# d3sm0/gym_pomdp

Hardware: AMD Instinct MI355X
Metric: env steps/sec (whole node), RockSample(7,8) batch=2^20, 1/2/4/8 MI355X (higher is better)
Workload: dtype int32

## Files before the change

### gym_pomdp_amd/csrc/envs/rock.hip.h

```cpp
#pragma once
#include "../envs_common.hip.h"

namespace pomdp {

template <int W, bool STOCH = false>
struct RockEnv {
    using Params = pomdp_rock_params;
    using Reward = int32_t;
    using S = typename std::conditional<W == 1, uint32_t, uint64_t>::type;
    static constexpr int WORDS = W;
    static constexpr const char *NAME = STOCH ? (W == 1 ? "StochasticRockEnv<1>" : "StochasticRockEnv<2>") : (W == 1 ? "RockEnv<1>" : "RockEnv<2>");
    static constexpr bool POOLED_LPT2 = !STOCH;
    static constexpr bool QUAD_STEP = true;
    static constexpr bool HAS_ROCKS = true;
    static constexpr bool POOLED_ANY_LPT = !STOCH;
    static constexpr bool STOCHASTIC = STOCH;
    static constexpr bool QUAD_TAB = true;
    struct Shared {
        uint2 thr[32];
        int8_t grid[256];
        uint8_t rxy[16];
        uint16_t rpos[16];
        uint32_t dir_y[16];
        uint32_t dir_x[16];
// ... 324 lines not shown
        const int penalty = STOCH ? 0 : -100;
        const int id = sh.grid[x * 16 + y];
        const int sh_ = 8 + 2 * (id & 15);
        const uint32_t code = (uint32_t)(s >> sh_) & 3u;
        const bool sample_ok = ((uint32_t)id < K) & (code != 1u);
        const uint32_t a2 = (uint32_t)a << 1;
        const uint32_t nx = x + (uint32_t)__builtin_amdgcn_sbfe(0xC4, a2, 2u), ny = y + (uint32_t)__builtin_amdgcn_sbfe(0x31, a2, 2u);
        const bool inside = max(nx, ny) < size;
        const bool is_move = a < 4, is_sample = a == 4, east = a == 1;
        const bool moved = is_move & inside, left = is_move & !inside, sampled = is_sample & sample_ok,
                   missed = is_sample & !sample_ok;
        const uint32_t d_move = ((uint32_t)s & 0xFFu) ^ (nx | (ny << 4));
        const S d_sample = (S)(code ^ 1u) << sh_;
        st.s = s ^ (moved ? (S)d_move : (sampled ? d_sample : (S)0));
        const bool good_rock = code == 2u;
        int rw = ((left & east) | (sampled & good_rock)) ? 10 : 0;
        rw = (sampled & !good_rock) ? -10 : rw;
        rw = ((left & !east) | missed) ? penalty : rw;
        rew = rw;
        if (STOCH) done = left & east;
        else done = left | missed;
    }
    static __device__ __forceinline__ uint32_t thr_lo_of(const Shared &sh, const State &st, int r)
    {
        const uint32_t x = (uint32_t)st.s & 15u, y = ((uint32_t)st.s >> 4) & 15u;
        return sh.thr[__builtin_amdgcn_sad_u8(x | (y << 8), sh.rpos[r & 15], 0u)].y;
    }
    static constexpr int TAB_ACTIONS = W == 1 ? 17 : 21;
    static __host__ __device__ __forceinline__ bool tab_ok(const Params &p) { return 5 + p.num_rocks <= TAB_ACTIONS; }

    static constexpr uint32_t REC_LUT_LO = 0x0A0A9CF6u, REC_LUT_HI = 0x00000000u;
    using TabEntry = typename std::conditional<W == 1, uint2, uint32_t>::type;
    struct RecTab { TabEntry e[TAB_ACTIONS][256]; };
    static constexpr uint32_t REC_ROCK = 1u << 31;
    static constexpr uint32_t TIE_SPAN = 32u;
    static __device__ __forceinline__ uint32_t rec_f(uint32_t off, int c, uint32_t ob_mask, uint32_t oc)
    {
        const uint32_t rbyte = (((uint64_t)REC_LUT_HI << 32 | REC_LUT_LO) >> (8u * oc)) & 0xFFu;
        return off | (((uint32_t)c & 3u) << 5) | (ob_mask << 8) | (rbyte << 16) | ((oc & 1u) << 24);
    }
    static __device__ __forceinline__ uint32_t rec_thr_word(uint32_t T) { return T >= (1u << 27) ? 0xFFFFFFFFu : T << 5; }
    template <uint32_t POS0 = 0u>
    static __device__ __forceinline__ void build_rec_tab(RecTab &tab, const Shared &sh, const Params &p, int pos)
    {
        constexpr uint32_t ROCK0 = (POS0 + 8u) & 31u;
        const uint32_t x = (uint32_t)pos & 15u, y = (uint32_t)pos >> 4, size = (uint32_t)p.size, K = (uint32_t)p.num_rocks;
        const int id = sh.grid[x * 16 + y];
        const uint32_t NOTHING = 6u << 28, PENALTY = (STOCH ? 6u : 1u) << 28, EXIT_EAST = 3u << 28;
        const uint32_t NO_TIE = 1u << 27;
        for (int a = 0; a < 5 + (int)K && a < TAB_ACTIONS; ++a) {
            uint32_t e, f;
            if (a < 4) {
                const uint32_t nx = x + (uint32_t)((a == 1) - (a == 3)), ny = y + (uint32_t)((a == 0) - (a == 2));
                const bool inside = max(nx, ny) < size;
                e = inside ? (((uint32_t)pos ^ (nx | (ny << 4))) | NOTHING) : (a == 1 ? EXIT_EAST : PENALTY);
                e |= NO_TIE;
                f = rec_f(POS0 + ((a & 1) ? 0u : 4u), inside ? (a < 2 ? 1 : -1) : 0, 0u, e >> 28 & 7u);
            } else if (a == 4) {
                const bool rock = (uint32_t)id < K;
                e = (rock ? ((8u + 2u * (uint32_t)id) | 0x80000000u) : 0u) | PENALTY | NO_TIE;
                f = rec_f(rock ? ROCK0 + 2u * (uint32_t)id : 0u, 0, 0u, e >> 28 & 7u);
            } else {
                e = sh.thr[__builtin_amdgcn_sad_u8(x | (y << 8), sh.rpos[a - 5], 0u) & 31u].x | NOTHING;
                f = rec_f(ROCK0 + 2u * (uint32_t)(a - 5), 0, 3u, 6u);
            }
            if constexpr (W == 1) tab.e[a][pos] = make_uint2(a > 4 ? rec_thr_word(e & ~NOTHING) : 0xFFFFFFFFu, f | (a == 4 ? e & REC_ROCK : 0u));
            else tab.e[a][pos] = e;
        }
    }
    template <class LowWord>
    static __device__ __forceinline__ bool sensor_exact_at(const Shared &sh, uint32_t xy, uint32_t r, uint32_t H, LowWord lo)
    {
        const uint2 t = sh.thr[__builtin_amdgcn_sad_u8(xy, sh.rpos[r], 0u) & 31u];
        const uint32_t kh = H >> 5;
        uint32_t kl = lo() >> 6;
        asm volatile("" : "+v"(kl));
        return kh == t.x ? kl <= t.y : kh < t.x;
    }

    static constexpr uint32_t ROT_POS = 24u;
    template <uint32_t POS0>
    struct Rec8 {
        static_assert(POS0 == 0u || POS0 == ROT_POS, "the memory layout, or the position byte on top");
        static constexpr uint32_t ROCK0 = (POS0 + 8u) & 31u;
        using Tab = RecTab;
        using Entry = uint2;
        static __device__ __forceinline__ uint32_t from_mem(uint32_t m) { return __builtin_amdgcn_alignbit(m, m, (32u - POS0) & 31u); }
        static __device__ __forceinline__ uint32_t to_mem(uint32_t s) { return __builtin_amdgcn_alignbit(s, s, POS0); }
        static __device__ __forceinline__ uint32_t start_word(uint32_t start) { return start << POS0; }
        static __device__ __forceinline__ bool builds(uint32_t) { return true; }
        static __device__ __forceinline__ void build(Tab &tab, const Shared &sh, const Params &p, int tid) { build_rec_tab<POS0>(tab, sh, p, tid); }
        static __device__ __forceinline__ Entry lookup(const Tab &tab, uint32_t s, uint32_t a)
        {
            if constexpr (POS0 == ROT_POS) {
                const uint32_t off = __builtin_amdgcn_alignbit(a, s, ROT_POS - 3u) & ~7u;
                return *reinterpret_cast<const uint2 *>(reinterpret_cast<const char *>(&tab.e[0][0]) + off);
            } else return tab.e[a][s & 0xFFu];
        }
        template <int N> static __device__ __forceinline__ void settle(Entry (&ef)[N])
        {
            uint64_t w[N];
#pragma unroll
            for (int j = 0; j < N; ++j) w[j] = (uint64_t)ef[j].x | ((uint64_t)ef[j].y << 32);
            if constexpr (N == 4) asm volatile("" : "+v"(w[0]), "+v"(w[1]), "+v"(w[2]), "+v"(w[3]));
            else asm volatile("" : "+v"(w[0]), "+v"(w[1]));
#pragma unroll
            for (int j = 0; j < N; ++j) ef[j] = make_uint2((uint32_t)w[j], (uint32_t)(w[j] >> 32));
        }
        static __device__ __forceinline__ uint32_t cmp(const Entry ef) { return ef.x; }
        template <class LowWord> static __device__ __forceinline__ bool exact(const Shared &sh, uint32_t s, const Entry ef, uint32_t H, LowWord lo)
        {
            const uint32_t pos = s >> POS0, r = (((ef.y & 31u) - ROCK0) >> 1) & 15u;
            return sensor_exact_at(sh, (pos & 15u) | ((pos & 0xF0u) << 4), r, H, lo);
        }
        template <class Act> static __device__ __forceinline__ void finish(const Entry ef, uint32_t &s, Act act, bool correct, uint32_t fresh, uint32_t &rec)
        {
            const uint32_t f = ef.y, a = act();
            const uint32_t q = __builtin_amdgcn_ubfe(s, f, 2u);
            const bool ok = ((int32_t)f < 0) & (q != 1u);
            const uint32_t keep = ((q == 2u) == correct) ? 0x7FFFFE00u : 0x7FFFFD00u;
            const uint32_t rfb = (f & keep) | a;
            const uint32_t rok = 0x00F60004u - q * 0x00760000u;
            rec = ok ? rok : rfb;
            const int c = ok ? 1 - (int)q : __builtin_amdgcn_sbfe((int)f, 5u, 2u);
            const uint32_t moved = s + ((uint32_t)c << (f & 31u));
            s = rec >= (1u << 24) ? fresh : moved;
        }
        static __device__ __forceinline__ uint32_t tie_bound(int) { return 0u; }
        template <int N> static __device__ __forceinline__ void fresh(const uint32_t (&R)[N], const RngKey &key, uint32_t first, int K, uint32_t start, uint32_t, uint32_t (&out)[N])
        {
            fresh_words<N, (int)ROCK0>(R, K, start, out);
            int fewest = __popc(R[0]);
#pragma unroll
            for (int e = 1; e < N; ++e) fewest = min(fewest, (int)__popc(R[e]));
            if (fewest <= 6) fresh_ties<N, (int)ROCK0>(R, key, first, K, out);
        }
    };
    using RecMem = Rec8<0u>;
    using RecRot = Rec8<ROT_POS>;

    static constexpr int WIDE_SIDE = 7;
    static __host__ __device__ __forceinline__ bool wide_ok(const Params &p) { return p.num_rocks <= RESET_NUMERIC_K && p.size <= WIDE_SIDE; }
    struct RecWide {
        static_assert(W == 1, "one state word");
        static constexpr int ACTIONS = 5 + RESET_NUMERIC_K, SLOTS = 128;
        static constexpr uint32_t X0 = 25u, Y0 = 28u, ROCK0 = 5u;
        struct Tab { u32x4 e[ACTIONS][SLOTS]; };
        using Entry = u32x4;
        static __device__ __forceinline__ uint32_t from_mem(uint32_t m) { return ((m & 7u) << X0) | ((m & 0x70u) << (Y0 - 4u)) | ((m >> (8u - ROCK0)) & (0xFFFFu << ROCK0)); }
        static __device__ __forceinline__ uint32_t to_mem(uint32_t s) { return ((s >> X0) & 7u) | ((s >> (Y0 - 4u)) & 0x70u) | ((s & (0xFFFFu << ROCK0)) << (8u - ROCK0)); }
        static __device__ __forceinline__ uint32_t start_word(uint32_t start) { return from_mem(start & 0xFFu); }
        static __device__ __forceinline__ uint32_t thr_word(uint32_t T) { return T >= (1u << 27) ? 0xFFFFFFE0u : T << 5; }
        static __device__ __forceinline__ bool builds(uint32_t tid) { return tid < (unsigned)SLOTS; }
        static __device__ __forceinline__ void build(Tab &tab, const Shared &sh, const Params &p, int slot)
        {
            const uint32_t x = (uint32_t)slot & 7u, y = ((uint32_t)slot >> 3) & 15u, size = (uint32_t)p.size, K = (uint32_t)p.num_rocks;
            const int id = sh.grid[x * 16 + y];
            const uint32_t penalty = STOCH ? 0u : (0x9Cu << 16) | (1u << 24);
            for (int a = 0; a < 5 + (int)K && a < ACTIONS; ++a) {
                uint32_t E = 0u, M = 0u, recA = (uint32_t)a, recB;
                if (a < 4) {
                    const uint32_t nx = x + (uint32_t)((a == 1) - (a == 3)), ny = y + (uint32_t)((a == 0) - (a == 2));
                    const uint32_t off = (a & 1) ? X0 : Y0;
                    if (max(nx, ny) < size) { E = ((a & 1) ? nx : ny) << off; M = 7u << off; }
                    else recA |= a == 1 ? (0x0Au << 16) | (1u << 24) : penalty;
                    recB = recA;
                } else if (a == 4) {
                    const uint32_t off = ROCK0 + 2u * (uint32_t)id;
                    if ((uint32_t)id < K) { E = 1u << off; M = (3u << off) | off | REC_ROCK; }
                    recA |= penalty;
                    recB = recA;
                } else {
                    E = thr_word(sh.thr[__builtin_amdgcn_sad_u8(x | (y << 8), sh.rpos[a - 5], 0u) & 31u].x);
                    M = ROCK0 + 2u * (uint32_t)(a - 5);
                    recB = recA | (1u << 8);
                    recA |= 2u << 8;
                }
                u32x4 e = {E, M, recA, recB};
                tab.e[a][slot] = e;
            }
        }
        static __device__ __forceinline__ Entry lookup(const Tab &tab, uint32_t s, uint32_t a)
        {
            const uint32_t off = __builtin_amdgcn_alignbit(a, s, X0 - 4u);
            return *reinterpret_cast<const u32x4 *>(reinterpret_cast<const char *>(&tab.e[0][0]) + off);
        }
        template <int N> static __device__ __forceinline__ void settle(Entry (&e)[N])
        {
            if constexpr (N == 4) asm volatile("" : "+v"(e[0]), "+v"(e[1]), "+v"(e[2]), "+v"(e[3]));
            else asm volatile("" : "+v"(e[0]), "+v"(e[1]));
        }
        static __device__ __forceinline__ uint32_t cmp(const Entry e) { return e.x; }
        template <class LowWord> static __device__ __forceinline__ bool exact(const Shared &sh, uint32_t s, const Entry e, uint32_t H, LowWord lo)
        {
            const uint32_t r = (((e.y & 31u) - ROCK0) >> 1) & 15u;
            return sensor_exact_at(sh, ((s >> X0) & 7u) | (((s >> Y0) & 7u) << 8), r, H, lo);
        }
        template <class Act> static __device__ __forceinline__ void finish(const Entry e, uint32_t &s, Act, bool correct, uint32_t fresh, uint32_t &rec)
        {
            const uint32_t M = e.y;
            const uint32_t q = __builtin_amdgcn_ubfe(s, M, 2u);
            const bool ok = ((int32_t)M < 0) & (q != 1u);
            const uint32_t rfb = ((q != 2u) != correct) ? e.z : e.w;
            const uint32_t rok = 0x00F60004u - q * 0x00760000u;
            rec = ok ? rok : rfb;
            uint32_t moved;
            asm("v_bfi_b32 %0, %1, %2, %3" : "=v"(moved) : "v"(M), "v"(e.x), "v"(s));
            asm("" : "+v"(rec));
            s = rec >= (1u << 24) ? fresh : moved;
        }
        static __device__ __forceinline__ uint32_t tie_bound(int K) { uint32_t b = 1u << (2 * min(K, RESET_NUMERIC_K) + 5); asm volatile("" : "+s"(b)); return b; }
        template <int N> static __device__ __forceinline__ void fresh(const uint32_t (&R)[N], const RngKey &key, uint32_t first, int K, uint32_t start, uint32_t bound, uint32_t (&out)[N])
        {
            fresh_words<N, (int)ROCK0>(R, K, start, out);
            uint32_t least = R[0];
#pragma unroll
            for (int e = 1; e < N; ++e) least = min(least, R[e]);
            if (least < bound) fresh_ties<N, (int)ROCK0>(R, key, first, K, out);
        }
    };
    template <class LowWord>
    static __device__ __forceinline__ void step_rec(const Shared &sh, const RecTab &tab, S &s, uint32_t a, uint32_t H, S fresh,
                                                    uint32_t &rec, LowWord lo)
    {
        const uint32_t s_lo = (uint32_t)s, s_hi = W == 2 ? (uint32_t)((uint64_t)s >> 32) : 0u;
        if constexpr (W == 1) {
            const auto ef = RecMem::lookup(tab, s_lo, a);
            bool correct = H < RecMem::cmp(ef);
            if (H - RecMem::cmp(ef) < TIE_SPAN) correct = RecMem::exact(sh, s_lo, ef, H, lo);
            uint32_t sn = s_lo;
            RecMem::finish(ef, sn, [&]() { return a; }, correct, (uint32_t)fresh, rec);
            s = (S)sn;
        } else {
            const uint32_t e = tab.e[a][s_lo & 0xFFu];
            const bool up_s = (e & 32u) != 0u;
            const uint32_t code = __builtin_amdgcn_ubfe(up_s ? s_hi : s_lo, e, 2u);
            const bool ok = ((int32_t)e < 0) & (code != 1u);
            const uint32_t collect = (code ^ 1u) << (e & 31u);
            const uint32_t move = (a < 4u ? e : 0u) & 0xFFu;
            const uint32_t d_lo = (ok & !up_s) ? collect : move, d_hi = (ok & up_s) ? collect : 0u;
            const uint32_t oc = ok ? code : __builtin_amdgcn_ubfe(e, 28u, 3u);
            const uint32_t rbyte = __builtin_amdgcn_perm(REC_LUT_HI, REC_LUT_LO, (oc << 16) | 0x0C000C0Cu);
            const uint32_t done = oc & 1u;
            const uint32_t gi = 2u * a - 1u;
            const bool good = __builtin_amdgcn_ubfe((gi & 32u) ? s_hi : s_lo, gi, 1u) != 0u;
            const uint32_t kh = __builtin_amdgcn_alignbit(12u, H, 5u);
            bool correct = kh < e;
            if (a > 4u && kh == e) correct = (lo() >> 6) <= thr_lo_of(sh, State{s}, (int)a - 5);
            const uint32_t ob = a > 4u ? ((good == correct) ? 2u << 8 : 1u << 8) : 0u;
            rec = rbyte | (done << 24) | ob | a;
            s = done ? fresh : (S)(((uint64_t)(s_hi ^ d_hi) << 32) | (s_lo ^ d_lo));
        }
    }

    template <class LowWord>
    static __device__ __forceinline__ int sensor_ob(const Shared &sh, const State &st, const Aux &aux, uint32_t H, LowWord lo)
    {
        const uint32_t kh = H >> 5;
        bool correct = kh < aux.th;
        if (kh == aux.th) correct = (lo() >> 6) <= thr_lo_of(sh, st, aux.r);
        return aux.want ? ((aux.good == correct) ? 2 : 1) : 0;
    }

    static constexpr bool QUAD_SENSOR = !STOCH;
    template <class RT>
    static __device__ __forceinline__ void step_with_H(const Shared &sh, const Params &p, State &st, int a, const RngKey &key,
                                                       uint32_t lane, uint32_t H, int &ob, RT &rew, int &done)
    {
        Aux aux;
        step_pre(sh, p, st, a, rew, done, aux);
        ob = sensor_ob(sh, st, aux, H, [&]() { return elem(quad_block(key, lane, 1u), lane & 3u); });
    }

    template <class RT>
    static __device__ __forceinline__ void step(const Shared &sh, const Params &p, State &st, int a,
                                                const RngKey &key, uint32_t lane, int &ob, RT &rew, int &done)
    {
        const uint32_t e = lane & 3u;
        if (STOCH) {
            const uint4 g = quad_block(key, lane, 0u);
            const bool act = k53_le(elem(g, e), (uint32_t)(p.act_thr >> 26), (uint32_t)p.act_thr & LO_MASK,
                                    [&]() { return elem(quad_block(key, lane, 1u), e); }) != (p.act_gt != 0);
            State nx = st;
            Aux aux; RT r2; int d2;
            step_pre(sh, p, nx, a, r2, d2, aux);
            const uint4 h = quad_block(key, lane, 2u);
            const int o2 = sensor_ob(sh, nx, aux, elem(h, e), [&]() { return elem(quad_block(key, lane, 3u), e); });
            if (act) { st = nx; rew = r2; done = d2; ob = o2; }
            else { rew = 0; done = 0; ob = 0; }
            return;
        }
        Aux aux;
        step_pre(sh, p, st, a, rew, done, aux);
        const uint4 h = quad_block(key, lane, 0u);
        ob = sensor_ob(sh, st, aux, elem(h, e), [&]() { return elem(quad_block(key, lane, 1u), e); });
    }
};

}
```

### gym_pomdp_amd/csrc/fused_impl.hip.h

```cpp
#pragma once
#include "kernels_common.hip.h"

namespace pomdp {

template <class L, bool TIGHT> constexpr bool hoist_fits = !(TIGHT && L::ID == LAYOUT_RETURNS);
template <class L, class Pol, int LPT = 4, bool SROW = false, bool HOIST = true>
struct FusedCtx {
    uint32_t l0, glane0;
    uint64_t t0;
    typename lanes_out<L, LPT, SROW>::type out;
    typename lanes_policy<Pol, LPT, HOIST>::type pol;
    uint32_t n_bad;
    __device__ __forceinline__ FusedCtx(int32_t *action, int32_t *ob, void *reward, uint8_t *done, int64_t rec, uint32_t lane0,
                                        const RngKey &key0, const RngKey &akey0, uint32_t n_act, int k_steps, const TapeRef &tape)
        : l0(blockIdx.x * (uint32_t)(LPT * BLOCK) + (uint32_t)LPT * threadIdx.x), glane0(lane0 + l0),
          t0(((uint64_t)key0.t_hi << 32) | key0.t_lo), out(action, ob, reward, done, rec, l0),
          pol(tape, l0, glane0, key0, akey0, n_act, k_steps), n_bad(0) {}
    __device__ __forceinline__ void first(int gen_first, int (&a_cur)[LPT])
    {
        if constexpr (LPT == 4) {
            const u32x4 a4 = out.first(pol, gen_first);
#pragma unroll
            for (int j = 0; j < 4; ++j) a_cur[j] = (int)a4[j];
        } else {
// ... 189 lines not shown
                const uint32_t rword = pick4(rq);
                st[0].s = fresh[0] ? Env::fresh_state(p, rword, key, glane[0]) : st[0].s;
            } else if constexpr (quad_word_env<Env>::value) {
                Env::fresh_w(sh, p, st[0], fresh[0], key, glane[0], pick4(sq));
            } else {
                Fin::resets_only(sh, p, st, fresh, key, glane);
            }
            const uint32_t word = pick4(aq);
            if constexpr (!TAPE) a_next[0] = (int)__umulhi(word, (uint32_t)n_act);
        } else {
            Fin::run(sh, p, st, fresh, key, glane, akey, (uint32_t)n_act, a_next, aux, o);
        }
#pragma unroll
        for (int j = 0; j < LPT; ++j) {
            if (!live[j]) { o[j] = 0; st[j] = before[j]; }
            if (in_range[j]) out.put_next_action(rel[j], a_next[j]);
            ever_fresh[j] |= fresh[j];
            if (in_range[j]) {
                uint32_t rcode = 0;
                if constexpr (L::CODES && !REC) rcode = Env::reward_code(r[j]);
                if constexpr (REC && L::CODES) out.put_record(j, rel[j], recv[j]);
                else out.put(j, rel[j], a_cur[j], o[j], r[j], rcode, d[j]);
                if (!valid[j] && !was_done[j] && err) atomicAdd(err, 1u);
            }
            if constexpr (TAPE4) a_next[j] = (int)tq[(std::decay_t<decltype(sj_)>::value + 1) & 3];
            else if constexpr (TAPE) a_next[j] = (int)col.nxt;
            a_cur[j] = a_next[j];
            was_done[j] = auto_reset ? false : (d[j] != 0);
        }
        out.next_row();
        if constexpr (Fin::LOOP_BARRIER && !quad_policy) __syncthreads();
    };
    if constexpr (UNROLL4 && UNROLL4_TAIL) {
        #pragma unroll 1
        for (int seg = 0, s = 0; seg < 4; ++seg) {
            const int seg_end = prio.template segment<4>(seg);
            #pragma unroll 1
            for (; s + 4 <= seg_end; s += 4) {
                step_body(s, std::integral_constant<int, 0>{});
                step_body(s + 1, std::integral_constant<int, 1>{});
                step_body(s + 2, std::integral_constant<int, 2>{});
                step_body(s + 3, std::integral_constant<int, 3>{});
            }
            #pragma unroll 1
            for (; s < seg_end; ++s) step_body(s, s & 3);
        }
    } else if constexpr (UNROLL4) {
        #pragma unroll 1
        for (int seg = 0, s = 0; seg < 4; ++seg)
        for (const int seg_end = prio.template segment<4>(seg); s < seg_end; s += 4) {
            step_body(s, std::integral_constant<int, 0>{});
            if (s + 1 < seg_end) {
                step_body(s + 1, std::integral_constant<int, 1>{});
                if (s + 2 < seg_end) {
                    step_body(s + 2, std::integral_constant<int, 2>{});
                    if (s + 3 < seg_end) step_body(s + 3, std::integral_constant<int, 3>{});
                }
            }
        }
    } else {
        #pragma unroll 1
        for (int seg = 0, s = 0; seg < 4; ++seg)
        for (const int seg_end = prio.segment(seg); s < seg_end; ++s) step_body(s, s & 3);
    }
#pragma unroll
    for (int j = 0; j < LPT; ++j)
        if (in_range[j]) { Env::store(st[j], state_w, n, rel[j], ever_fresh[j]); out.finish(j, rel[j], k_steps); }
}

template <class Env, class L, class Pol, int LPT, class Form>
__device__ __forceinline__ void steps_quad_body(uint32_t *__restrict__ state, int32_t *__restrict__ action,
                                                int32_t *__restrict__ ob, int32_t *__restrict__ reward,
                                                uint8_t *__restrict__ done, int64_t n, RngKey key0, uint32_t lane0,
                                                RngKey akey0, int k_steps, int64_t rec, int gen_first,
                                                const typename Env::Params &p, TapeRef tape)
{
    static_assert(LPT == 4 || LPT == 2, "a quad or half a quad per thread");
    constexpr int W = Env::WORDS;
    using S = typename Env::S;
    __shared__ typename Env::Shared sh;
    __shared__ typename Form::Tab tab;
    const uint32_t n_act = (uint32_t)Env::n_actions(p);
    constexpr bool AHEAD2 = Pol::TAPE && LPT == 4;
    using PolT = typename std::conditional<AHEAD2, TapeQuadAhead, Pol>::type;
    constexpr bool HOIST = hoist_fits<L, Env::STOCHASTIC>;
    FusedCtx<L, PolT, LPT, true, HOIST> cx(action, ob, reward, done, rec, lane0, key0, akey0, n_act, k_steps, tape);
    const uint32_t l0 = cx.l0, glane0 = cx.glane0;
    const uint32_t e0 = LPT == 4 ? 0u : (glane0 & 2u);
    typename Env::State st[LPT];
    int a_cur[LPT];
    uint32_t sp0 = 0, sp1 = 0, gp0 = 0, gp1 = 0;
    {
        uint32_t s_lo[LPT], s_hi[LPT];
        if constexpr (LPT == 4) {
            const u32x4 lo = ld_stream4(state + l0);
            u32x4 hi = {0, 0, 0, 0};
            if (W == 2) hi = ld_stream4(state + n + l0);
#pragma unroll
            for (int j = 0; j < 4; ++j) { s_lo[j] = lo[j]; s_hi[j] = hi[j]; }
        } else {
            const u32x2 lo = ld_stream2(state + l0);
            u32x2 hi = {0, 0};
            if (W == 2) hi = ld_stream2(state + n + l0);
#pragma unroll
            for (int j = 0; j < 2; ++j) { s_lo[j] = lo[j]; s_hi[j] = hi[j]; }
        }
        cx.first(gen_first, a_cur);
#pragma unroll
        for (int j = 0; j < LPT; ++j) {
            if constexpr (W == 1) st[j].s = Form::from_mem(s_lo[j]);
            else st[j].s = (S)((uint64_t)s_lo[j] | ((uint64_t)s_hi[j] << 32));
        }
    }
    Env::stage(sh, p, (int)threadIdx.x);
    __syncthreads();
    if constexpr (W == 1) { if (Form::builds(threadIdx.x)) Form::build(tab, sh, p, (int)threadIdx.x); }
    else Env::build_rec_tab(tab, sh, p, (int)threadIdx.x);
    __syncthreads();
    const int K = p.num_rocks;
    const uint32_t start = (uint32_t)p.start_x | ((uint32_t)p.start_y << 4);
    uint32_t start_rot = start, tie_bound = 0;
    if constexpr (W == 1) { start_rot = Form::start_word(start); asm volatile("" : "+v"(start_rot)); }
    const LoopPrio prio(k_steps);
    constexpr uint32_t SENSOR_BLOCK = Env::SENSOR_BLOCK;
    constexpr int NFX = AHEAD2 ? 2 : 1;
    PhiloxFixed sensor_fx[NFX], gate_fx[NFX];
#pragma unroll
    for (int h = 0; h < NFX; ++h) {
        sensor_fx[h] = philox_fixed(glane0 >> 2, ((uint32_t)POMDP_STREAM_STEP << 24) | SENSOR_BLOCK, key0.k1);
        gate_fx[h] = philox_fixed(glane0 >> 2, (uint32_t)POMDP_STREAM_STEP << 24, key0.k1);
    }
    auto stretch = [&](const int s, int end) __attribute__((always_inline)) {
        end = cx.stretch(s, end);
        if constexpr (LPT == 4 && HOIST) {
#pragma unroll
            for (int h = 0; h < NFX; ++h) {
                const RngKey kh = cx.key(key0, s + h);
                philox_hoist(sensor_fx[h], kh.t_hi, kh.k0);
                if constexpr (Env::STOCHASTIC) philox_hoist(gate_fx[h], kh.t_hi, kh.k0);
                end = stretch_end<NFX>(s, end, kh.t_lo);
            }
        }
        return end;
    };
    if constexpr (W == 1) tie_bound = Form::tie_bound(K);
    auto step_body = [&](const int s, const auto par_) __attribute__((always_inline)) {
        constexpr int PAR = decltype(par_)::value;
        const RngKey key = cx.key(key0, s);
        uint32_t H[LPT], G[LPT];
        if constexpr (LPT == 4) {
            const uint4 sw = philox4x32_10_fixed<HOIST>(sensor_fx[AHEAD2 ? PAR : 0], key.t_lo, key.t_hi, key.k0, key.k1);
            H[0] = sw.x; H[1] = sw.y; H[2] = sw.z; H[3] = sw.w;
        } else {
            pair_shared(s, e0 != 0u, [&](int sb) { return Env::quad_block(cx.key(key0, sb), glane0, SENSOR_BLOCK); }, H, sp0, sp1);
        }
        uint32_t a_next[LPT];
        if constexpr (AHEAD2) cx.pol.template begin_par<PAR>(s, a_next);
        else cx.pol.begin(s, a_next);
        bool acts[LPT];
#pragma unroll
        for (int j = 0; j < LPT; ++j) acts[j] = true;
        if constexpr (Env::STOCHASTIC) {
            if constexpr (LPT == 4) {
                const uint4 gw = philox4x32_10_fixed<HOIST>(gate_fx[AHEAD2 ? PAR : 0], key.t_lo, key.t_hi, key.k0, key.k1);
                G[0] = gw.x; G[1] = gw.y; G[2] = gw.z; G[3] = gw.w;
            } else {
                pair_shared(s, e0 != 0u, [&](int sb) { return Env::quad_block(cx.key(key0, sb), glane0, 0u); }, G, gp0, gp1);
            }
#pragma unroll
            for (int j = 0; j < LPT; ++j)
                acts[j] = Env::k53_le(G[j], (uint32_t)(p.act_thr >> 26), (uint32_t)p.act_thr & Env::LO_MASK,
                                      [&]() { return Env::elem(Env::quad_block(key, glane0, 1u), e0 + (uint32_t)j); }) != (p.act_gt != 0);
        }
        uint32_t rec[LPT], a_taken[LPT];
#pragma unroll
        for (int j = 0; j < LPT; ++j) a_taken[j] = (uint32_t)a_cur[j];
        bool valid[LPT];
#pragma unroll
        for (int j = 0; j < LPT; ++j) valid[j] = !Pol::TAPE || a_taken[j] < n_act;
        auto low_word = [&](int j) __attribute__((always_inline)) {
            return Env::elem(Env::quad_block(rare_key(key), glane0 + (uint32_t)j, SENSOR_BLOCK + 1u), e0 + (uint32_t)j);
        };
        if constexpr (W == 1) {
            uint32_t fresh[LPT], sn[LPT];
            typename Form::Entry ef[LPT];
            Form::template fresh<LPT>(H, key, glane0, K, start_rot, tie_bound, fresh);
#pragma unroll
            for (int j = 0; j < LPT; ++j) ef[j] = Form::lookup(tab, st[j].s, valid[j] ? a_taken[j] : 0u);
            Form::template settle<LPT>(ef);
            uint32_t near[LPT];
            bool correct[LPT];
#pragma unroll
            for (int j = 0; j < LPT; ++j) correct[j] = __builtin_sub_overflow(H[j], Form::cmp(ef[j]), &near[j]);
            uint32_t nearest = near[0];
#pragma unroll
            for (int j = 1; j < LPT; ++j) nearest = min(nearest, near[j]);
            if (nearest < Env::TIE_SPAN) {
#pragma unroll
                for (int j = 0; j < LPT; ++j)
                    if (near[j] < Env::TIE_SPAN) correct[j] = Form::exact(sh, st[j].s, ef[j], H[j], [&]() { return low_word(j); });
            }
#pragma unroll
            for (int j = 0; j < LPT; ++j) {
                sn[j] = st[j].s;
                Form::finish(ef[j], sn[j], [&]() { return valid[j] ? a_taken[j] : 0u; }, correct[j], fresh[j], rec[j]);
            }
#pragma unroll
            for (int j = 0; j < LPT; ++j) {
                if constexpr (Env::STOCHASTIC) {
                    sn[j] = acts[j] ? sn[j] : st[j].s;
                    rec[j] = acts[j] ? rec[j] : a_taken[j];
                }
                if constexpr (Pol::TAPE) {
                    sn[j] = valid[j] ? sn[j] : st[j].s;
                    rec[j] = valid[j] ? rec[j] : a_taken[j];
                    cx.n_bad += (uint32_t)!valid[j];
                }
                st[j].s = sn[j];
            }
        } else {
            uint32_t codes[LPT];
            if constexpr (LPT == 4) Env::reset_codes4(H, key, glane0, K, codes);
            else {
#pragma unroll
                for (int j = 0; j < LPT; ++j) codes[j] = Env::template reset_codes<true>(H[j], key, glane0 + (uint32_t)j, K);
            }
#pragma unroll
            for (int j = 0; j < LPT; ++j) {
                S sj = st[j].s;
                Env::step_rec(sh, tab, sj, valid[j] ? a_taken[j] : 0u, H[j], (S)((uint64_t)start | ((uint64_t)codes[j] << 8)), rec[j],
                              [&]() { return low_word(j); });
                if constexpr (Env::STOCHASTIC) {
                    sj = acts[j] ? sj : st[j].s;
                    rec[j] = acts[j] ? rec[j] : a_taken[j];
                }
                if constexpr (Pol::TAPE) {
                    sj = valid[j] ? sj : st[j].s;
                    rec[j] = valid[j] ? rec[j] : a_taken[j];
                    cx.n_bad += (uint32_t)!valid[j];
                }
                st[j].s = sj;
            }
        }
        cx.out.put_records(rec, a_next);
        if constexpr (AHEAD2) {
            cx.pol.template end_par<PAR>(s, a_next);
#pragma unroll
            for (int j = 0; j < LPT; ++j) a_cur[j] = (int)a_next[j];
        } else cx.advance(s, a_next, a_cur);
    };
    if constexpr (AHEAD2) {
        wait_loads();
        _Pragma("unroll 1") for (int seg = 0, s = 0; seg < 4; ++seg)
            _Pragma("unroll 1") for (const int seg_end = prio.template segment<2>(seg); s < seg_end;)
                _Pragma("unroll 1") for (const int end = stretch(s, seg_end); s < end; s += 2) {
                    step_body(s, std::integral_constant<int, 0>{});
                    if (s + 1 < end) step_body(s + 1, std::integral_constant<int, 1>{});
                }
    } else {
        POMDP_FUSED_STEP_LOOP(prio, s, stretch) step_body(s, std::integral_constant<int, 0>{});
    }
    cx.finish(k_steps);
    uint32_t w_lo[LPT];
#pragma unroll
    for (int j = 0; j < LPT; ++j) {
        w_lo[j] = (uint32_t)st[j].s;
        if constexpr (W == 1) w_lo[j] = Form::to_mem(w_lo[j]);
    }
    if constexpr (LPT == 4) {
        st_stream4(state + l0, w_lo[0], w_lo[1], w_lo[2], w_lo[3]);
        if (W == 2)
            st_stream4(state + n + l0, (uint32_t)((uint64_t)st[0].s >> 32), (uint32_t)((uint64_t)st[1].s >> 32),
                       (uint32_t)((uint64_t)st[2].s >> 32), (uint32_t)((uint64_t)st[3].s >> 32));
    } else {
        st_stream2(state + l0, w_lo[0], w_lo[1]);
        if (W == 2) st_stream2(state + n + l0, (uint32_t)((uint64_t)st[0].s >> 32), (uint32_t)((uint64_t)st[1].s >> 32));
    }
}
template <class Env, class L = Columns, class Pol = SyntheticQuad, int LPT = 4>
__global__ __launch_bounds__(BLOCK) void steps_quad_kernel(uint32_t *__restrict__ state, int32_t *__restrict__ action,
                                                           int32_t *__restrict__ ob, int32_t *__restrict__ reward,
                                                           uint8_t *__restrict__ done, int64_t n, RngKey key0, uint32_t lane0,
                                                           RngKey akey0, int k_steps, int64_t rec, int gen_first,
                                                           const typename Env::Params p, TapeRef tape)
{
    using Form = typename std::conditional<Env::WORDS == 1, typename Env::RecWide, typename Env::RecMem>::type;
    steps_quad_body<Env, L, Pol, LPT, Form>(state, action, ob, reward, done, n, key0, lane0, akey0, k_steps, rec, gen_first, p, tape);
}
template <class Env, class L = Columns, class Pol = SyntheticQuad, int LPT = 4>
__global__ __launch_bounds__(BLOCK) void steps_quad_popc_kernel(uint32_t *__restrict__ state, int32_t *__restrict__ action,
                                                                int32_t *__restrict__ ob, int32_t *__restrict__ reward,
                                                                uint8_t *__restrict__ done, int64_t n, RngKey key0, uint32_t lane0,
                                                                RngKey akey0, int k_steps, int64_t rec, int gen_first,
                                                                const typename Env::Params p, TapeRef tape)
{
    static_assert(Env::WORDS == 1, "two state words take steps_quad_kernel");
    steps_quad_body<Env, L, Pol, LPT, typename Env::RecRot>(state, action, ob, reward, done, n, key0, lane0, akey0, k_steps, rec, gen_first, p, tape);
}

template <bool TAB, class L = Columns, class Pol = SyntheticQuad, int LPT = 4>
__global__ __launch_bounds__(BLOCK) void tag_steps_quad_kernel(uint32_t *__restrict__ state, int32_t *__restrict__ action,
                                                               int32_t *__restrict__ ob, float *__restrict__ reward,
                                                               uint8_t *__restrict__ done, int64_t n, RngKey key0,
                                                               uint32_t lane0, RngKey akey0, int k_steps, int64_t rec,
                                                               int gen_first, const TagEnv::Params p, TapeRef tape)
{
    using Env = TagEnv;
    static_assert(LPT == 4 || LPT == 2, "a quad or half a quad per thread");
    __shared__ Env::Shared sh;
    __shared__ typename std::conditional<TAB, Env::StepTab, NoTab>::type tab;
    const uint32_t n_act = (uint32_t)Env::n_actions(p);
    FusedCtx<L, Pol, LPT, false, L::ID != POMDP_LAYOUT_NARROW> cx(action, ob, reward, done, rec, lane0, key0, akey0, n_act, k_steps, tape);
    const uint32_t l0 = cx.l0, glane0 = cx.glane0;
    const uint32_t e0 = LPT == 4 ? 0u : (glane0 & 2u);
    Env::State st[LPT];
    int a_cur[LPT];
    uint32_t sp0 = 0, sp1 = 0;
    {
        if constexpr (LPT == 4) {
            const u32x4 s4 = ld_stream4(state + l0);
            cx.first(gen_first, a_cur);
#pragma unroll
            for (int j = 0; j < 4; ++j) st[j].w = s4[j];
        } else {
            const u32x2 s2 = ld_stream2(state + l0);
            cx.first(gen_first, a_cur);
#pragma unroll
            for (int j = 0; j < 2; ++j) st[j].w = s2[j];
        }
    }
    Env::stage(sh, p, (int)threadIdx.x);
    __syncthreads();
    if constexpr (TAB) {
        Env::build_tab(tab, sh, p, (int)threadIdx.x);
        __syncthreads();
    }
    const LoopPrio prio(k_steps);
    POMDP_FUSED_STEP_LOOP(prio, s, cx.stretch) {
        const RngKey key = cx.key(key0, s);
        uint32_t a_next[LPT];
        cx.pol.begin(s, a_next);
        int o[LPT], d[LPT];
        float r[LPT];
        uint32_t a_taken[LPT], W[LPT];
#pragma unroll
        for (int j = 0; j < LPT; ++j) a_taken[j] = (uint32_t)a_cur[j];
        if constexpr (LPT == 4) {
            const uint4 qw = Env::quad_block(key, glane0, 0u);
            W[0] = qw.x; W[1] = qw.y; W[2] = qw.z; W[3] = qw.w;
        } else {
            pair_shared(s, e0 != 0u, [&](int sb) { return Env::quad_block(cx.key(key0, sb), glane0, 0u); }, W, sp0, sp1);
        }
#pragma unroll
        for (int j = 0; j < LPT; ++j) {
            Env::Flight f;
            const bool valid = !Pol::TAPE || a_taken[j] < n_act;
            const Env::State before = st[j];
            const int a = valid ? a_cur[j] : 0;
            if constexpr (TAB) Env::step_one_opponent_tab(tab, st[j], a, o[j], r[j], d[j], f);
            else Env::step_one_opponent_pre(sh, p, st[j], a, o[j], r[j], d[j], f);
            const uint32_t lane = glane0 + (uint32_t)j;
            if constexpr (Pol::TAPE) { if (!valid) { f.need = false; o[j] = 0; r[j] = 0.f; d[j] = 0; cx.n_bad++; } }
            Env::flee_word(sh, p, st[j], f, W[j], [&]() { return Env::elem(Env::quad_block(key, lane, 1u), e0 + (uint32_t)j); });
            if (d[j]) Env::auto_reset_word(p, st[j], W[j], key, lane);
            if constexpr (Pol::TAPE) st[j] = valid ? st[j] : before;
        }
        uint32_t o4[LPT], r4[LPT], d4[LPT], rc[LPT];
#pragma unroll
        for (int j = 0; j < LPT; ++j) {
// ... 707 lines not shown
```

### gym_pomdp_amd/csrc/traj_out.hip.h

```cpp
#pragma once
#include "envs.hip.h"

namespace pomdp {

constexpr int LAYOUT_RETURNS = 100;
template <bool ACT> struct ColumnsT { static constexpr int ID = POMDP_LAYOUT_COLUMNS; static constexpr const char *NAME = "Columns"; static constexpr bool CODES = false; };
using Columns = ColumnsT<true>;
using ColumnsNoAct = ColumnsT<false>;
struct Blocked { static constexpr int ID = POMDP_LAYOUT_BLOCKED; static constexpr const char *NAME = "Blocked"; static constexpr bool CODES = false; };
struct Packed  { static constexpr int ID = POMDP_LAYOUT_PACKED;  static constexpr const char *NAME = "Packed";  static constexpr bool CODES = true; };
struct Narrow  { static constexpr int ID = POMDP_LAYOUT_NARROW;  static constexpr const char *NAME = "Narrow";  static constexpr bool CODES = true; };
template <class Env> struct Returns { static constexpr int ID = LAYOUT_RETURNS; static constexpr const char *NAME = "Returns"; static constexpr bool CODES = true; using E = Env; };

constexpr int TRAJ_BLOCK_LANES = 256;
constexpr int TRAJ_BLOCK_BYTES = 13 * TRAJ_BLOCK_LANES;

static __device__ __forceinline__ uint32_t pack_record(uint32_t a, uint32_t o, uint32_t rcode, uint32_t d)
{
    return a | (o << 8) | ((rcode & 0xFFu) << 16) | (d << 24);
}

struct TapeRef {
    const uint8_t *base;
    int64_t stride;
    uint32_t *err;
};

template <class T>
struct TapeColumn {
    const uint8_t *p;
    int64_t stride;
    int last;
    T first, nxt;
    __device__ __forceinline__ T row(int r) const
    {
        r = r < last ? r : last;
        return ld_stream(reinterpret_cast<const T *>(p + (int64_t)r * stride));
    }
    __device__ __forceinline__ TapeColumn(const TapeRef &t, uint32_t col, int k_steps)
        : p(t.base + col), stride(t.stride), last(k_steps - 1), nxt(0) { first = row(0); }
    __device__ __forceinline__ void request(int s) { nxt = row(s + 1); }
};
struct NoColumn {
    uint8_t first, nxt;
    __device__ __forceinline__ NoColumn(const TapeRef &, uint32_t, int) : first(0), nxt(0) {}
    __device__ __forceinline__ void request(int) {}
};

template <bool HOIST>
struct SyntheticQuadT {
    static constexpr bool TAPE = false;
    uint32_t glane0, n_act, k0, k1;
    uint64_t ta0;
    PhiloxFixed fx;
    __device__ __forceinline__ SyntheticQuadT(const TapeRef &, uint32_t, uint32_t glane0_, const RngKey &key0, const RngKey &akey0, uint32_t n_act_, int)
        : glane0(glane0_), n_act(n_act_), k0(key0.k0), k1(key0.k1), ta0(((uint64_t)akey0.t_hi << 32) | akey0.t_lo),
          fx(philox_fixed(glane0_ >> 2, (uint32_t)POMDP_STREAM_ACTION << 24, key0.k1)) {}
    __device__ __forceinline__ int stretch(int s, int end)
    {
        if constexpr (!HOIST) return end;
        const uint64_t ta = ta0 + (uint64_t)s;
        philox_hoist(fx, (uint32_t)(ta >> 32), k0);
        return stretch_end(s, end, (uint32_t)ta);
    }
    __device__ __forceinline__ uint4 block(uint64_t ta) const
    {
        return philox4x32_10_fixed<HOIST>(fx, (uint32_t)ta, (uint32_t)(ta >> 32), k0, k1);
    }
    __device__ __forceinline__ u32x4 first() const
    {
        const uint64_t ta = ta0 - 1ull;
        const uint4 w = philox4x32_10_fixed<false>(fx, (uint32_t)ta, (uint32_t)(ta >> 32), k0, k1);
        return u32x4{__umulhi(w.x, n_act), __umulhi(w.y, n_act), __umulhi(w.z, n_act), __umulhi(w.w, n_act)};
    }
    __device__ __forceinline__ void begin(int s, uint32_t (&a)[4]) const
    {
        const uint4 pw = block(ta0 + (uint64_t)s);
        a[0] = __umulhi(pw.x, n_act); a[1] = __umulhi(pw.y, n_act); a[2] = __umulhi(pw.z, n_act); a[3] = __umulhi(pw.w, n_act);
    }
    __device__ __forceinline__ void end(int, uint32_t (&)[4]) const {}
    __device__ __forceinline__ void count_bad(uint32_t) const {}
};
struct SyntheticQuad : SyntheticQuadT<true> { using SyntheticQuadT<true>::SyntheticQuadT; };
struct SyntheticQuadPlain : SyntheticQuadT<false> { using SyntheticQuadT<false>::SyntheticQuadT; };
struct TapeQuad {
    static constexpr bool TAPE = true;
    TapeColumn<uint32_t> col;
    uint32_t *err;
    static __device__ __forceinline__ void unpack(uint32_t w, uint32_t (&a)[4])
    {
        a[0] = w & 0xFFu; a[1] = __builtin_amdgcn_ubfe(w, 8u, 8u); a[2] = __builtin_amdgcn_ubfe(w, 16u, 8u); a[3] = w >> 24;
    }
    __device__ __forceinline__ TapeQuad(const TapeRef &t, uint32_t l0, uint32_t, const RngKey &, const RngKey &, uint32_t, int k_steps)
        : col(t, l0, k_steps), err(t.err) {}
    __device__ __forceinline__ u32x4 first() const
    {
        uint32_t a[4];
        unpack(col.first, a);
        return u32x4{a[0], a[1], a[2], a[3]};
    }
    __device__ __forceinline__ void begin(int s, uint32_t (&a)[4]) { col.request(s); a[0] = a[1] = a[2] = a[3] = 0; }
    __device__ __forceinline__ void end(int, uint32_t (&a)[4]) const { unpack(col.nxt, a); }
    __device__ __forceinline__ void count_bad(uint32_t n_bad) const { if (n_bad && err) atomicAdd(err, n_bad); }
    __device__ __forceinline__ int stretch(int, int end) const { return end; }
};

struct TapeQuadAhead {
    static constexpr bool TAPE = true;
    TapeColumn<uint32_t> col;
    uint32_t *err;
    uint32_t even, odd;
    __device__ __forceinline__ TapeQuadAhead(const TapeRef &t, uint32_t l0, uint32_t, const RngKey &, const RngKey &, uint32_t, int k_steps)
        : col(t, l0, k_steps), err(t.err), even(0), odd(col.row(1)) {}
    __device__ __forceinline__ u32x4 first() const
    {
        uint32_t a[4];
        TapeQuad::unpack(col.first, a);
        return u32x4{a[0], a[1], a[2], a[3]};
    }
    template <int PAR> __device__ __forceinline__ void begin_par(int s, uint32_t (&a)[4])
    {
        if constexpr (PAR == 0) even = col.row(s + 2); else odd = col.row(s + 2);
        a[0] = a[1] = a[2] = a[3] = 0;
    }
    template <int PAR> __device__ __forceinline__ void end_par(int, uint32_t (&a)[4]) const { TapeQuad::unpack(PAR == 0 ? odd : even, a); }
    __device__ __forceinline__ void count_bad(uint32_t n_bad) const { if (n_bad && err) atomicAdd(err, n_bad); }
    __device__ __forceinline__ int stretch(int, int end) const { return end; }
};

static __device__ __forceinline__ uint32_t pair_swap(uint32_t v)
{
    return (uint32_t)__builtin_amdgcn_update_dpp((int)v, (int)v, 0xB1, 0xF, 0xF, false);
}
template <class BlockOfStep>
static __device__ __forceinline__ void pair_shared(int s, bool hi, BlockOfStep block_of_step, uint32_t (&w)[2], uint32_t &odd0, uint32_t &odd1)
{
    if ((s & 1) == 0) {
        const uint4 b = block_of_step(s + (hi ? 1 : 0));
        const uint32_t r0 = pair_swap(hi ? b.x : b.z), r1 = pair_swap(hi ? b.y : b.w);
        w[0] = hi ? r0 : b.x; w[1] = hi ? r1 : b.y;
        odd0 = hi ? b.z : r0; odd1 = hi ? b.w : r1;
    } else { w[0] = odd0; w[1] = odd1; }
}
struct SyntheticPair {
    static constexpr bool TAPE = false;
    uint32_t glane0, n_act, k0, k1, odd[2];
    uint64_t ta0;
    bool hi;
    __device__ __forceinline__ SyntheticPair(const TapeRef &, uint32_t, uint32_t glane0_, const RngKey &key0, const RngKey &akey0, uint32_t n_act_, int)
        : glane0(glane0_), n_act(n_act_), k0(key0.k0), k1(key0.k1), odd{0, 0}, ta0(((uint64_t)akey0.t_hi << 32) | akey0.t_lo), hi((glane0_ & 2u) != 0u) {}
    __device__ __forceinline__ uint4 block(uint64_t ta) const
    {
        return philox4x32_10(glane0 >> 2, (uint32_t)ta, (uint32_t)(ta >> 32), (uint32_t)POMDP_STREAM_ACTION << 24, k0, k1);
    }
    __device__ __forceinline__ void first(uint32_t (&a)[2]) const
    {
        const uint4 w = block(ta0 - 1ull);
        a[0] = __umulhi(hi ? w.z : w.x, n_act); a[1] = __umulhi(hi ? w.w : w.y, n_act);
    }
    __device__ __forceinline__ void begin(int s, uint32_t (&a)[2])
    {
        if ((s & 1) == 0) {
            const uint4 w = block(ta0 + (uint64_t)s + (hi ? 1ull : 0ull));
            const uint32_t r0 = pair_swap(hi ? w.x : w.z), r1 = pair_swap(hi ? w.y : w.w);
            a[0] = __umulhi(hi ? r0 : w.x, n_act); a[1] = __umulhi(hi ? r1 : w.y, n_act);
            odd[0] = __umulhi(hi ? w.z : r0, n_act); odd[1] = __umulhi(hi ? w.w : r1, n_act);
        } else { a[0] = odd[0]; a[1] = odd[1]; }
    }
    __device__ __forceinline__ void end(int, uint32_t (&)[2]) const {}
    __device__ __forceinline__ void count_bad(uint32_t) const {}
    __device__ __forceinline__ int stretch(int, int end) const { return end; }
};
struct TapePair {
    static constexpr bool TAPE = true;
    TapeColumn<uint16_t> col;
    uint32_t *err;
    __device__ __forceinline__ TapePair(const TapeRef &t, uint32_t l0, uint32_t, const RngKey &, const RngKey &, uint32_t, int k_steps)
        : col(t, l0, k_steps), err(t.err) {}
    __device__ __forceinline__ void first(uint32_t (&a)[2]) const { a[0] = col.first & 0xFFu; a[1] = (uint32_t)col.first >> 8; }
    __device__ __forceinline__ void begin(int s, uint32_t (&a)[2]) { col.request(s); a[0] = a[1] = 0; }
    __device__ __forceinline__ void end(int, uint32_t (&a)[2]) const { a[0] = col.nxt & 0xFFu; a[1] = (uint32_t)col.nxt >> 8; }
    __device__ __forceinline__ void count_bad(uint32_t n_bad) const { if (n_bad && err) atomicAdd(err, n_bad); }
    __device__ __forceinline__ int stretch(int, int end) const { return end; }
};
template <class Pol, int LPT, bool HOIST = true> struct lanes_policy { using type = Pol; };
template <bool HOIST> struct lanes_policy<SyntheticQuad, 2, HOIST> { using type = SyntheticPair; };
template <bool HOIST> struct lanes_policy<TapeQuad, 2, HOIST> { using type = TapePair; };
template <> struct lanes_policy<SyntheticQuad, 4, false> { using type = SyntheticQuadPlain; };

template <class L> struct QuadOut;

static __device__ __forceinline__ void unpack_records(const uint32_t (&rec)[4], uint32_t (&a)[4], uint32_t (&o)[4], uint32_t (&r)[4], uint32_t (&d)[4])
{
#pragma unroll
    for (int j = 0; j < 4; ++j) {
        a[j] = rec[j] & 0xFFu;
        o[j] = __builtin_amdgcn_ubfe(rec[j], 8u, 8u);
        r[j] = (uint32_t)__builtin_amdgcn_sbfe(rec[j], 16u, 8u);
        d[j] = rec[j] >> 24;
    }
}

template <bool ACT> struct QuadOut<ColumnsT<ACT>> {
    uint32_t *action_w, *ob_w, *reward_w, *done_w;
    int64_t rec;
    __device__ __forceinline__ QuadOut(void *action, void *ob, void *reward, void *done, int64_t rec_, uint32_t l0)
        : action_w(ACT ? reinterpret_cast<uint32_t *>(action) + l0 : nullptr), ob_w(reinterpret_cast<uint32_t *>(ob) + l0),
          reward_w(reinterpret_cast<uint32_t *>(reward) + l0), done_w(reinterpret_cast<uint32_t *>(reinterpret_cast<uint8_t *>(done) + l0)),
// ... 490 lines not shown
```

Measured before the change: 1030 billion.

## Add no-op table row for tape actions and reschedule tape prefetch

Adds an extra all-zero row to the wide RockSample transition table for tape-driven packed/narrow layouts. Out-of-range tape actions now look up that no-op row instead of going through per-lane validity selects, and bad actions are counted only when the largest action is out of range. The tape prefetch is also restructured: the next-next row load is issued after the current row is unpacked, three steps ahead, and the even/odd step pair is run unconditionally with a tail step for odd counts. The aim is less selection work and more load/compute overlap, at the cost of a larger shared table and more prefetch registers.

Result: no change. 1033 billion, median of 3 (+0.3%).

```diff
diff --git a/gym_pomdp_amd/csrc/envs/rock.hip.h b/gym_pomdp_amd/csrc/envs/rock.hip.h
--- a/gym_pomdp_amd/csrc/envs/rock.hip.h
+++ b/gym_pomdp_amd/csrc/envs/rock.hip.h
@@ -430,6 +430,7 @@
     template <uint32_t POS0>
     struct Rec8 {
         static_assert(POS0 == 0u || POS0 == ROT_POS, "the memory layout, or the position byte on top");
+        static constexpr bool NOOP_ROW = false;
         static constexpr uint32_t ROCK0 = (POS0 + 8u) & 31u;
         using Tab = RecTab;
         using Entry = uint2;
@@ -493,21 +494,25 @@
         static_assert(W == 1, "one state word");
         static constexpr int ACTIONS = 5 + RESET_NUMERIC_K, SLOTS = 128;
         static constexpr uint32_t X0 = 25u, Y0 = 28u, ROCK0 = 5u;
-        struct Tab { u32x4 e[ACTIONS][SLOTS]; };
+        static constexpr bool NOOP_ROW = false;
+        template <int ROWS> struct TabOf { u32x4 e[ROWS][SLOTS]; };
+        using Tab = TabOf<ACTIONS>;
         using Entry = u32x4;
         static __device__ __forceinline__ uint32_t from_mem(uint32_t m) { return ((m & 7u) << X0) | ((m & 0x70u) << (Y0 - 4u)) | ((m >> (8u - ROCK0)) & (0xFFFFu << ROCK0)); }
         static __device__ __forceinline__ uint32_t to_mem(uint32_t s) { return ((s >> X0) & 7u) | ((s >> (Y0 - 4u)) & 0x70u) | ((s & (0xFFFFu << ROCK0)) << (8u - ROCK0)); }
         static __device__ __forceinline__ uint32_t start_word(uint32_t start) { return from_mem(start & 0xFFu); }
         static __device__ __forceinline__ uint32_t thr_word(uint32_t T) { return T >= (1u << 27) ? 0xFFFFFFE0u : T << 5; }
         static __device__ __forceinline__ bool builds(uint32_t tid) { return tid < (unsigned)SLOTS; }
-        static __device__ __forceinline__ void build(Tab &tab, const Shared &sh, const Params &p, int slot)
+        template <int ROWS> static __device__ __forceinline__ void build(TabOf<ROWS> &tab, const Shared &sh, const Params &p, int slot)
         {
             const uint32_t x = (uint32_t)slot & 7u, y = ((uint32_t)slot >> 3) & 15u, size = (uint32_t)p.size, K = (uint32_t)p.num_rocks;
             const int id = sh.grid[x * 16 + y];
             const uint32_t penalty = STOCH ? 0u : (0x9Cu << 16) | (1u << 24);
-            for (int a = 0; a < 5 + (int)K && a < ACTIONS; ++a) {
+            constexpr int EXTRA = ROWS > ACTIONS ? 1 : 0;
+            for (int a = 0; a < 5 + (int)K + EXTRA && a < ACTIONS + EXTRA; ++a) {
                 uint32_t E = 0u, M = 0u, recA = (uint32_t)a, recB;
-                if (a < 4) {
+                if (EXTRA && a == 5 + (int)K) recA = recB = 0u;
+                else if (a < 4) {
                     const uint32_t nx = x + (uint32_t)((a == 1) - (a == 3)), ny = y + (uint32_t)((a == 0) - (a == 2));
                     const uint32_t off = (a & 1) ? X0 : Y0;
                     if (max(nx, ny) < size) { E = ((a & 1) ? nx : ny) << off; M = 7u << off; }
@@ -528,7 +533,7 @@
                 tab.e[a][slot] = e;
             }
         }
-        static __device__ __forceinline__ Entry lookup(const Tab &tab, uint32_t s, uint32_t a)
+        template <int ROWS> static __device__ __forceinline__ Entry lookup(const TabOf<ROWS> &tab, uint32_t s, uint32_t a)
         {
             const uint32_t off = __builtin_amdgcn_alignbit(a, s, X0 - 4u);
             return *reinterpret_cast<const u32x4 *>(reinterpret_cast<const char *>(&tab.e[0][0]) + off);
@@ -566,6 +571,12 @@
             for (int e = 1; e < N; ++e) least = min(least, R[e]);
             if (least < bound) fresh_ties<N, (int)ROCK0>(R, key, first, K, out);
         }
+    };
+    struct RecWideTape : RecWide {
+        static constexpr int ACTIONS = RecWide::ACTIONS + 1;
+        static constexpr bool NOOP_ROW = true;
+        using Tab = typename RecWide::template TabOf<ACTIONS>;
+        static_assert(ACTIONS == 5 + RESET_NUMERIC_K + 1, "wide_ok: at most RESET_NUMERIC_K rocks, and the row after their CHECKs");
     };
     template <class LowWord>
     static __device__ __forceinline__ void step_rec(const Shared &sh, const RecTab &tab, S &s, uint32_t a, uint32_t H, S fresh,
diff --git a/gym_pomdp_amd/csrc/fused_impl.hip.h b/gym_pomdp_amd/csrc/fused_impl.hip.h
--- a/gym_pomdp_amd/csrc/fused_impl.hip.h
+++ b/gym_pomdp_amd/csrc/fused_impl.hip.h
@@ -295,7 +295,9 @@
     __shared__ typename Form::Tab tab;
     const uint32_t n_act = (uint32_t)Env::n_actions(p);
     constexpr bool AHEAD2 = Pol::TAPE && LPT == 4;
-    using PolT = typename std::conditional<AHEAD2, TapeQuadAhead, Pol>::type;
+    constexpr bool EARLY = AHEAD2 && (L::ID == POMDP_LAYOUT_PACKED || L::ID == POMDP_LAYOUT_NARROW);
+    using PolT = typename std::conditional<AHEAD2, TapeQuadAhead<EARLY>, Pol>::type;
+    constexpr bool NOOP = Pol::TAPE && Form::NOOP_ROW;
     constexpr bool HOIST = hoist_fits<L, Env::STOCHASTIC>;
     FusedCtx<L, PolT, LPT, true, HOIST> cx(action, ob, reward, done, rec, lane0, key0, akey0, n_act, k_steps, tape);
     const uint32_t l0 = cx.l0, glane0 = cx.glane0;
@@ -357,8 +359,9 @@
         return end;
     };
     if constexpr (W == 1) tie_bound = Form::tie_bound(K);
-    auto step_body = [&](const int s, const auto par_) __attribute__((always_inline)) {
+    auto step_body = [&](const int s, const auto par_, const auto more_) __attribute__((always_inline)) {
         constexpr int PAR = decltype(par_)::value;
+        constexpr bool MORE = decltype(more_)::value;
         const RngKey key = cx.key(key0, s);
         uint32_t H[LPT], G[LPT];
         if constexpr (LPT == 4) {
@@ -368,7 +371,7 @@
             pair_shared(s, e0 != 0u, [&](int sb) { return Env::quad_block(cx.key(key0, sb), glane0, SENSOR_BLOCK); }, H, sp0, sp1);
         }
         uint32_t a_next[LPT];
-        if constexpr (AHEAD2) cx.pol.template begin_par<PAR>(s, a_next);
+        if constexpr (AHEAD2) cx.pol.template top<PAR>(s);
         else cx.pol.begin(s, a_next);
         bool acts[LPT];
 #pragma unroll
@@ -390,7 +393,7 @@
         for (int j = 0; j < LPT; ++j) a_taken[j] = (uint32_t)a_cur[j];
         bool valid[LPT];
 #pragma unroll
-        for (int j = 0; j < LPT; ++j) valid[j] = !Pol::TAPE || a_taken[j] < n_act;
+        for (int j = 0; j < LPT; ++j) valid[j] = !Pol::TAPE || NOOP || a_taken[j] < n_act;
         auto low_word = [&](int j) __attribute__((always_inline)) {
             return Env::elem(Env::quad_block(rare_key(key), glane0 + (uint32_t)j, SENSOR_BLOCK + 1u), e0 + (uint32_t)j);
         };
@@ -399,7 +402,7 @@
             typename Form::Entry ef[LPT];
             Form::template fresh<LPT>(H, key, glane0, K, start_rot, tie_bound, fresh);
 #pragma unroll
-            for (int j = 0; j < LPT; ++j) ef[j] = Form::lookup(tab, st[j].s, valid[j] ? a_taken[j] : 0u);
+            for (int j = 0; j < LPT; ++j) ef[j] = Form::lookup(tab, st[j].s, NOOP ? min(a_taken[j], n_act) : valid[j] ? a_taken[j] : 0u);
             Form::template settle<LPT>(ef);
             uint32_t near[LPT];
             bool correct[LPT];
@@ -424,12 +427,22 @@
                     sn[j] = acts[j] ? sn[j] : st[j].s;
                     rec[j] = acts[j] ? rec[j] : a_taken[j];
                 }
-                if constexpr (Pol::TAPE) {
+                if constexpr (NOOP) rec[j] |= a_taken[j];
+                else if constexpr (Pol::TAPE) {
                     sn[j] = valid[j] ? sn[j] : st[j].s;
                     rec[j] = valid[j] ? rec[j] : a_taken[j];
                     cx.n_bad += (uint32_t)!valid[j];
                 }
                 st[j].s = sn[j];
+            }
+            if constexpr (NOOP) {
+                uint32_t largest = a_taken[0];
+#pragma unroll
+                for (int j = 1; j < LPT; ++j) largest = max(largest, a_taken[j]);
+                if (largest >= n_act) {
+#pragma unroll
+                    for (int j = 0; j < LPT; ++j) cx.n_bad += (uint32_t)(a_taken[j] >= n_act);
+                }
             }
         } else {
             uint32_t codes[LPT];
@@ -455,23 +468,39 @@
                 st[j].s = sj;
             }
         }
-        cx.out.put_records(rec, a_next);
         if constexpr (AHEAD2) {
-            cx.pol.template end_par<PAR>(s, a_next);
+            cx.pol.template arrive<PAR, MORE>(s, a_next);
+            cx.out.put_records(rec, a_next);
 #pragma unroll
             for (int j = 0; j < LPT; ++j) a_cur[j] = (int)a_next[j];
-        } else cx.advance(s, a_next, a_cur);
+        } else {
+            cx.out.put_records(rec, a_next);
+            cx.advance(s, a_next, a_cur);
+        }
     };
-    if constexpr (AHEAD2) {
+    if constexpr (EARLY) {
+        wait_loads();
+        const int k_even = k_steps & ~1;
+        _Pragma("unroll 1") for (int seg = 0, s = 0; seg < 4; ++seg)
+            _Pragma("unroll 1") for (const int seg_end = min(prio.template segment<2>(seg), k_even); s < seg_end;)
+                _Pragma("unroll 1") for (const int end = stretch(s, seg_end); s < end; s += 2) {
+                    step_body(s, std::integral_constant<int, 0>{}, std::true_type{});
+                    step_body(s + 1, std::integral_constant<int, 1>{}, std::true_type{});
+                }
+        if (k_steps & 1) {
+            stretch(k_even, k_steps);
+            step_body(k_even, std::integral_constant<int, 0>{}, std::false_type{});
+        }
+    } else if constexpr (AHEAD2) {
         wait_loads();
         _Pragma("unroll 1") for (int seg = 0, s = 0; seg < 4; ++seg)
             _Pragma("unroll 1") for (const int seg_end = prio.template segment<2>(seg); s < seg_end;)
                 _Pragma("unroll 1") for (const int end = stretch(s, seg_end); s < end; s += 2) {
-                    step_body(s, std::integral_constant<int, 0>{});
-                    if (s + 1 < end) step_body(s + 1, std::integral_constant<int, 1>{});
+                    step_body(s, std::integral_constant<int, 0>{}, std::true_type{});
+                    if (s + 1 < end) step_body(s + 1, std::integral_constant<int, 1>{}, std::true_type{});
                 }
     } else {
-        POMDP_FUSED_STEP_LOOP(prio, s, stretch) step_body(s, std::integral_constant<int, 0>{});
+        POMDP_FUSED_STEP_LOOP(prio, s, stretch) step_body(s, std::integral_constant<int, 0>{}, std::true_type{});
     }
     cx.finish(k_steps);
     uint32_t w_lo[LPT];
@@ -497,7 +526,9 @@
                                                            RngKey akey0, int k_steps, int64_t rec, int gen_first,
                                                            const typename Env::Params p, TapeRef tape)
 {
-    using Form = typename std::conditional<Env::WORDS == 1, typename Env::RecWide, typename Env::RecMem>::type;
+    constexpr bool TAPE_ROW = Pol::TAPE && (L::ID == POMDP_LAYOUT_PACKED || L::ID == POMDP_LAYOUT_NARROW);
+    using Wide = typename std::conditional<TAPE_ROW, typename Env::RecWideTape, typename Env::RecWide>::type;
+    using Form = typename std::conditional<Env::WORDS == 1, Wide, typename Env::RecMem>::type;
     steps_quad_body<Env, L, Pol, LPT, Form>(state, action, ob, reward, done, n, key0, lane0, akey0, k_steps, rec, gen_first, p, tape);
 }
 template <class Env, class L = Columns, class Pol = SyntheticQuad, int LPT = 4>
diff --git a/gym_pomdp_amd/csrc/traj_out.hip.h b/gym_pomdp_amd/csrc/traj_out.hip.h
--- a/gym_pomdp_amd/csrc/traj_out.hip.h
+++ b/gym_pomdp_amd/csrc/traj_out.hip.h
@@ -105,25 +105,34 @@
     __device__ __forceinline__ int stretch(int, int end) const { return end; }
 };
 
+template <bool STORES>
 struct TapeQuadAhead {
     static constexpr bool TAPE = true;
     TapeColumn<uint32_t> col;
     uint32_t *err;
     uint32_t even, odd;
     __device__ __forceinline__ TapeQuadAhead(const TapeRef &t, uint32_t l0, uint32_t, const RngKey &, const RngKey &, uint32_t, int k_steps)
-        : col(t, l0, k_steps), err(t.err), even(0), odd(col.row(1)) {}
+        : col(t, l0, k_steps), err(t.err), even(STORES ? col.row(2) : 0u), odd(col.row(1)) {}
     __device__ __forceinline__ u32x4 first() const
     {
         uint32_t a[4];
         TapeQuad::unpack(col.first, a);
         return u32x4{a[0], a[1], a[2], a[3]};
     }
-    template <int PAR> __device__ __forceinline__ void begin_par(int s, uint32_t (&a)[4])
-    {
-        if constexpr (PAR == 0) even = col.row(s + 2); else odd = col.row(s + 2);
-        a[0] = a[1] = a[2] = a[3] = 0;
-    }
-    template <int PAR> __device__ __forceinline__ void end_par(int, uint32_t (&a)[4]) const { TapeQuad::unpack(PAR == 0 ? odd : even, a); }
+    template <int PAR> __device__ __forceinline__ void top(int s)
+    {
+        if constexpr (!STORES) { if constexpr (PAR == 0) even = col.row(s + 2); else odd = col.row(s + 2); }
+    }
+    template <int PAR, bool MORE> __device__ __forceinline__ void arrive(int s, uint32_t (&a)[4])
+    {
+        uint32_t &reg = PAR == 0 ? odd : even;
+        TapeQuad::unpack(reg, a);
+        if constexpr (STORES && MORE) {
+            int r = s + 3;
+            asm("" : "+s"(r) : "v"(a[0]), "v"(a[1]), "v"(a[2]), "v"(a[3]));
+            reg = col.row(r);
+        }
+    }
     __device__ __forceinline__ void count_bad(uint32_t n_bad) const { if (n_bad && err) atomicAdd(err, n_bad); }
     __device__ __forceinline__ int stretch(int, int end) const { return end; }
 };
```
